# andimarafioti/faster-qwen3-tts

Measured on AMD Instinct MI355X. Metric: real-time factor (audio s / wall s), Qwen3-TTS-12Hz-0.6B voice-clone streaming chunk_size=8; p50 TTFA in ttfa_ms_p50, higher is better.
Workload: dtype bf16

## Files before the change

faster-qwen3-tts_amd/csrc/decode_kernels.cuh:

```cuda
#pragma once
#include "fq3_common.cuh"
#include <initializer_list>

namespace fq3 {

enum { PRO_PLAIN = 0, PRO_NORM = 1, PRO_COMBINE = 2 };
enum { EPI_STORE = 0, EPI_RESIDUAL = 1, EPI_SWIGLU = 2 };

constexpr int kHeadDim = 128;
constexpr int kKeysPerTile = 64;
constexpr int kMaxWorkers = 8;
constexpr int kPartStride = kHeadDim + 4;


struct GemvArgs {
    const void* W; int N; int K;
    const void* x;
    const void* norm_w; float eps;
    const void* bias;
    void* y;
    const void* res;
    void* xn_out;
    int up_off;
    const float* part; int n_part; int rep;
// ... 236 lines not shown
    a.norm_w = norm_w; a.eps = eps; a.up_off = up_off; a.n_part = n_part; a.rep = rep;
    a.bias = t.bias; a.y = t.y; a.res = t.res; a.xn_out = t.xn_out;
    a.x2 = t.x2; a.y2 = t.y2; a.res2 = t.res2; a.part_stride2 = t.part_stride2;
    gemv_body<T, NCH, PRO, EPI, NT, M, R>(a);
}
template <typename T, int NCH, int PRO, int EPI, bool NT, int M, int R>
inline void gemv_launch(const GemvArgs& a, int grid, size_t shm, hipStream_t s) {
    const GemvTail t{a.y, a.res, a.bias, a.xn_out, a.x2, a.y2, a.res2, a.part_stride2};
    const void* x = PRO == PRO_COMBINE ? static_cast<const void*>(a.part) : a.x;
    hipLaunchKernelGGL((gemv_kernel<T, NCH, PRO, EPI, NT, M, R>), dim3(grid), dim3(256), shm, s, a.W, x, a.norm_w, a.N, a.K, a.eps, a.up_off,
                       a.n_part, a.rep, t);
}

struct AttnArgs {
    const void* qkv;
    const void* q_norm_w; const void* k_norm_w; float eps;
    const float* cos_row; const float* sin_row;
    void* kcache; void* vcache; int max_seq;
    const int* table; int blk_stride;
    const int* pos_ptr; int pos_imm; int n_pad;
    const int* done_ptr;
    int n_kv; float* part; float scale;
    int rep; void* out;
};

template <typename T, int REP, bool PAGED>
__device__ __forceinline__ void attn_decode_body(const AttnArgs& a) {
    constexpr int HD = kHeadDim, KS = kKeysPerTile, NG = KS / 16;
    const int g = blockIdx.x, s = blockIdx.y, S = gridDim.y;
    __shared__ float qs[REP][HD];
    __shared__ float knew[HD], vnew[HD];
    __shared__ float wo[4][REP][HD];
    __shared__ float wm[4][REP], wl[4][REP];
    const int tid = threadIdx.x, wave = tid >> 6, lane = tid & 63;
    const int sub = lane >> 4, c = lane & 15;
    const T* qkv = reinterpret_cast<const T*>(a.qkv);
    const int q_dim = a.n_kv * REP * HD, kv_dim = a.n_kv * HD;
    T* kc = reinterpret_cast<T*>(a.kcache) + (PAGED ? (size_t)g * KS * HD : (size_t)g * a.max_seq * HD);
    T* vc = reinterpret_cast<T*>(a.vcache) + (PAGED ? (size_t)g * KS * HD : (size_t)g * a.max_seq * HD);
    const int n_tiles = (a.max_seq + KS - 1) / KS;
    auto block_of = [&](int tile) -> int {
        if constexpr (PAGED) return a.table[tile < n_tiles ? tile : n_tiles - 1];
        else return 0;
    };
    int blk = block_of(s), blk_next = block_of(s + S);

// ... 123 lines not shown
        }
    }
    __syncthreads();
    for (int e = tid; e < REP * HD; e += 256) {
        const int h = e / HD, d = e - h * HD;
        float M = fmaxf(fmaxf(wm[0][h], wm[1][h]), fmaxf(wm[2][h], wm[3][h]));
        float num = 0.f, den = 0.f;
#pragma unroll
        for (int w = 0; w < 4; ++w) {
            const float ww = __expf(wm[w][h] - M);
            num = fmaf(ww, wo[w][h][d], num);
            den = fmaf(ww, wl[w][h], den);
        }
        float* p = a.part + (((size_t)g * kMaxWorkers + s) * REP + h) * kPartStride;
        p[d] = num;
        if (d == 0) { p[HD] = M; p[HD + 1] = den; }
    }
}

struct AttnTail {
    const void* q_norm_w; const void* k_norm_w; const float* cos_row; const float* sin_row;
    const int* table; const int* pos_ptr; const int* done_ptr; float* part; void* out;
    float eps; float scale; int n_pad; int blk_stride; int rep;
};
inline AttnTail attn_tail(const AttnArgs& a) {
    return AttnTail{a.q_norm_w, a.k_norm_w, a.cos_row, a.sin_row, a.table, a.pos_ptr, a.done_ptr, a.part, a.out, a.eps, a.scale, a.n_pad, a.blk_stride, a.rep};
}
__device__ __forceinline__ AttnArgs attn_args_of(const AttnTail& t) {
    AttnArgs a;
    a.q_norm_w = t.q_norm_w; a.k_norm_w = t.k_norm_w; a.cos_row = t.cos_row; a.sin_row = t.sin_row;
    a.table = t.table; a.pos_ptr = t.pos_ptr; a.done_ptr = t.done_ptr; a.part = t.part; a.out = t.out;
    a.eps = t.eps; a.scale = t.scale; a.n_pad = t.n_pad; a.blk_stride = t.blk_stride; a.rep = t.rep;
    return a;
}

constexpr int kAttnDecodeLeadDwords = 14;
template <typename T, int REP, bool PAGED>
__global__ __launch_bounds__(256) void attn_decode_kernel(const int* table, const void* qkv, void* kcache, void* vcache, const int* pos_ptr,
                                                          int max_seq, int n_kv, int blk_stride, int pos_imm, AttnTail t) {
    AttnArgs a = attn_args_of(t);
    a.table = table; a.qkv = qkv; a.kcache = kcache; a.vcache = vcache; a.pos_ptr = pos_ptr;
    a.max_seq = max_seq; a.n_kv = n_kv; a.blk_stride = blk_stride; a.pos_imm = pos_imm;
    attn_decode_body<T, REP, PAGED>(a);
}
template <typename T, int REP, bool PAGED>
inline void attn_decode_launch(const AttnArgs& a, int workers, hipStream_t s) {
    hipLaunchKernelGGL((attn_decode_kernel<T, REP, PAGED>), dim3(a.n_kv, workers), dim3(256), 0, s, a.table, a.qkv, a.kcache, a.vcache, a.pos_ptr,
                       a.max_seq, a.n_kv, a.blk_stride, a.pos_imm, attn_tail(a));
}

template <typename T>
__device__ __forceinline__ void attn_pred_body(const AttnArgs& a, int head) {
    constexpr int HD = kHeadDim;
    const int g = head / a.rep, hh = head - g * a.rep;
    const int lane = threadIdx.x & 63, sub = lane >> 4, c = lane & 15;
    const int pos = a.pos_imm;
    const T* qkv = reinterpret_cast<const T*>(a.qkv);
    const int q_dim = a.n_kv * a.rep * HD, kv_dim = a.n_kv * HD;
    T* kc = reinterpret_cast<T*>(a.kcache) + (size_t)g * a.max_seq * HD;
    T* vc = reinterpret_cast<T*>(a.vcache) + (size_t)g * a.max_seq * HD;
    Raw8<T> qraw, knraw, vnraw, qwraw, kwraw, kr[4], vr[4];
    ldraw<false>(qraw, qkv + (size_t)head * HD + c * 8);
    ldraw<false>(knraw, qkv + q_dim + (size_t)g * HD + c * 8);
    ldraw<false>(vnraw, qkv + q_dim + kv_dim + (size_t)g * HD + c * 8);
    ldraw<false>(qwraw, reinterpret_cast<const T*>(a.q_norm_w) + c * 8);
    ldraw<false>(kwraw, reinterpret_cast<const T*>(a.k_norm_w) + c * 8);
    const f32x4 cs0 = *reinterpret_cast<const f32x4*>(a.cos_row + ((c * 8) & 63)), cs1 = *reinterpret_cast<const f32x4*>(a.cos_row + ((c * 8 + 4) & 63));
    const f32x4 sn0 = *reinterpret_cast<const f32x4*>(a.sin_row + ((c * 8) & 63)), sn1 = *reinterpret_cast<const f32x4*>(a.sin_row + ((c * 8 + 4) & 63));
#pragma unroll
    for (int i = 0; i < 4; ++i) {
        int key = i * 4 + sub;
        key = key < a.max_seq ? key : a.max_seq - 1;
        ldraw<false>(kr[i], kc + (size_t)key * HD + c * 8);
        ldraw<false>(vr[i], vc + (size_t)key * HD + c * 8);
    }
    __builtin_amdgcn_sched_barrier(0);
    const float sgn = c < 8 ? -1.f : 1.f;
    const float cs[8] = {cs0.x, cs0.y, cs0.z, cs0.w, cs1.x, cs1.y, cs1.z, cs1.w};
    const float sn[8] = {sgn * sn0.x, sgn * sn0.y, sgn * sn0.z, sgn * sn0.w, sgn * sn1.x, sgn * sn1.y, sgn * sn1.z, sgn * sn1.w};
    auto norm_rope = [&](const Raw8<T>& raw, const Raw8<T>& wraw, float (&out)[8]) {
#pragma clang fp contract(off)
        float x[8], w[8];
        unpack(raw, x); unpack(wraw, w);
        float ss = 0.f;
#pragma unroll
        for (int i = 0; i < 8; ++i) ss = fmaf(x[i], x[i], ss);
        ss = row16_sum(ss);
        const float rs = 1.0f / sqrtf(ss / (float)HD + a.eps);
#pragma unroll
        for (int i = 0; i < 8; i += 2) {
            float u = x[i] * rs, v = x[i + 1] * rs;
            DT<T>::rnd2(u, v);
            u *= w[i]; v *= w[i + 1];
            DT<T>::rnd2(u, v);
            x[i] = u; x[i + 1] = v;
        }
#pragma unroll
        for (int i = 0; i < 8; i += 2) {
// ... 319 lines not shown
```

faster-qwen3-tts_amd/csrc/fq3_api.hip:

```cpp
#define FQ3_SKINNY_EXTERN
#include "fq3_ctx.h"
#include "sampler.cuh"
#include "sampler_wave.cuh"
#include "skinny_gemm.cuh"
#include "state_kernels.cuh"

#include <cstdio>
#include <cstdlib>
#include <cstring>
#include <map>
#include <string>
#include <type_traits>
#include <vector>

using namespace fq3;

static thread_local std::string g_err;
static int fail(int code, const std::string& m) { g_err = m; return code; }
int fq3_fail_(int code, const std::string& m) { return fail(code, m); }
#define HIPCHK(x) do { hipError_t e_ = (x); if (e_ != hipSuccess) return fail(FQ3_EHIP, std::string(#x) + ": " + hipGetErrorString(e_)); } while (0)

extern "C" const char* fq3_last_error(void) { return g_err.c_str(); }
extern "C" void fq3_set_error_(const char* msg) { g_err = msg ? msg : ""; }
extern "C" int fq3_abi_version(void) { return FQ3_ABI_VERSION; }

static int dmalloc(fq3_ctx* c, void** p, size_t bytes, bool zero = true) {
    HIPCHK(hipMalloc(p, bytes));
    if (zero) HIPCHK(hipMemset(*p, 0, bytes));
    c->allocs.push_back(*p);
// ... 184 lines not shown
    if ((r = dmalloc(c, &c->act2, (size_t)Im * c->esz))) return r;
    if ((r = dmalloc(c, &c->pred_x2, (size_t)p.hidden * c->esz))) return r;
    if ((r = dmalloc(c, &c->xin, (size_t)Hm * c->esz))) return r;
    if ((r = dmalloc(c, &c->tmp_hidden, (size_t)Hm * c->esz))) return r;
    if ((r = dmalloc(c, &c->qkv, (size_t)qkvm * c->esz))) return r;
    if ((r = dmalloc(c, &c->act, (size_t)Im * c->esz))) return r;
    if ((r = dmalloc(c, &c->logits, (size_t)Vm * c->esz))) return r;
    if ((r = dmalloc(c, &c->past_hidden, (size_t)t.hidden * c->esz))) return r;
    if ((r = dmalloc(c, &c->ph_hold, (size_t)t.hidden * c->esz))) return r;
    if ((r = dmalloc(c, &c->pred_in, (size_t)2 * t.hidden * c->esz))) return r;
    if ((r = dmalloc(c, &c->pred_next, (size_t)t.hidden * c->esz))) return r;
    if ((r = dmalloc(c, &c->pred_x, (size_t)p.hidden * c->esz))) return r;
    if ((r = dmalloc(c, &c->plogits, (size_t)(G - 1) * p.vocab * c->esz))) return r;
    const int maxkv = std::max(t.n_kv_heads, p.n_kv_heads);
    c->part_stride = (size_t)maxkv * kMaxWorkers * 4 * kPartStride;
    if ((r = dmalloc(c, (void**)&c->part, 2 * c->part_stride * sizeof(float)))) return r;
    if ((r = dmalloc(c, (void**)&c->rope_now, 2 * 64 * sizeof(float)))) return r;
    if ((r = dmalloc(c, (void**)&c->seen_api, kMaxVocab))) return r;
    if ((r = dmalloc(c, (void**)&c->st, sizeof(DecodeState)))) return r;
    if ((r = dmalloc(c, (void**)&c->seen, kMaxVocab))) return r;
    if ((r = dmalloc(c, (void**)&c->codes, (size_t)(frames + 1) * G * sizeof(int)))) return r;
    if ((r = dmalloc(c, (void**)&c->ids64, (size_t)64 * sizeof(int64_t)))) return r;
    if ((r = dmalloc(c, (void**)&c->d_pemb, (size_t)64 * sizeof(void*)))) return r;
    HIPCHK(hipStreamCreateWithFlags(&c->cap_stream, hipStreamNonBlocking));
    return FQ3_OK;
}

extern "C" int fq3_set_option(fq3_ctx* c, const char* key, int value) {
    if (!c || !key) return fail(FQ3_EINVAL, "null argument");
    const std::string k(key);
    if (k == "weight_nt") c->opt_nt = value;
    else if (k == "pred_m2") c->opt_m2 = value;
    else if (k == "pred_attn") c->opt_pred_attn = value;
    else if (k == "rows_per_wave_max") c->opt_rmax = value;
    else if (k == "prefill_mode") c->prefill_mode = value;
    else if (k == "flash_prefill") c->opt_flash_prefill = value;
    else if (k == "flash_small") c->opt_flash_small = value;
    else if (k == "cont_pack") c->opt_cont_pack = value;
    else if (k == "swiglu_tile") c->opt_swiglu_tile = value;
    else if (k == "packed_weights") c->opt_packed = value;
    else if (k == "skinny_gemm") c->opt_no_skinny = !value;
    else return fail(FQ3_EINVAL, "unknown option: " + k);
    fq3_graph_reset(c);
    return FQ3_OK;
}

extern "C" int fq3_graph_reset(fq3_ctx* c) {
    if (!c) return fail(FQ3_EINVAL, "null ctx");
    if (c->exec) { (void)hipGraphExecDestroy(c->exec); c->exec = nullptr; }
    if (c->graph) { (void)hipGraphDestroy(c->graph); c->graph = nullptr; }
    return FQ3_OK;
}

namespace {
struct PackedEntry { void* p; int refs; int N, K; };
std::mutex g_packed_mu;
std::map<std::pair<const void*, int>, PackedEntry> g_packed;
// ... 35 lines not shown
        const int r = fq3_packed_acquire_(W, N, K, kind);
        if (r == FQ3_OK) c->packed_refs.emplace_back(W, kind);
        return r == FQ3_EUNSUPPORTED ? FQ3_OK : r;
    };
    auto stack = [&](const std::vector<fq3_layer_weights>& L, const fq3_stack_dims& d) -> int {
        const int qd = d.n_heads * kHeadDim, kvd = d.n_kv_heads * kHeadDim;
        for (const fq3_layer_weights& l : L) {
            if (int r = take(l.qkv, qd + 2 * kvd, d.hidden, 0)) return r;
            if (int r = take(l.o, d.hidden, qd, 0)) return r;
            if (int r = take(l.gate_up, 2 * d.inter, d.hidden, 1)) return r;
            if (int r = take(l.gate_up, 2 * d.inter, d.hidden, 0)) return r;
            if (int r = take(l.down, d.hidden, d.inter, 0)) return r;
        }
        return FQ3_OK;
    };
    if (int r = stack(c->tl, c->cfg.talker)) return r;
    if (int r = stack(c->pl, c->cfg.predictor)) return r;
    for (const fq3_layer_weights& l : c->tl) if (int r = take(l.gate_up, 2 * c->cfg.talker.inter, c->cfg.talker.hidden, 2)) return r;
    if (int r = take(c->wt.codec_head, c->cfg.talker.vocab, c->cfg.talker.hidden, 0)) return r;
    for (const void* h : c->lmh) if (int r = take(h, c->cfg.predictor.vocab, c->cfg.predictor.hidden, 0)) return r;
    return FQ3_OK;
}

extern "C" int fq3_ctx_destroy(fq3_ctx* c) {
    if (!c) return FQ3_OK;
    (void)hipDeviceSynchronize();
    fq3_graph_reset(c);
    packed_release_all(c);
    if (c->cap_stream) (void)hipStreamDestroy(c->cap_stream);
    if (fq3_kv_pool* p = c->tk.pool) {
        (void)fq3_kv_release(c, 0);
        bool last;
        { std::lock_guard<std::mutex> lk(p->mu); last = --p->users == 0; }
        if (p->is_private && last) pool_free_(p);
    }
    for (void* p : c->allocs) (void)hipFree(p);
    delete c;
    return FQ3_OK;
}

extern "C" int fq3_bind_weights(fq3_ctx* c, const fq3_weight_table* w) {
    if (!c || !w) return fail(FQ3_EINVAL, "null argument");
    const int G = c->cfg.num_code_groups;
    if (!w->talker_layers || !w->predictor_layers || !w->codec_embedding || !w->codec_head || !w->talker_final_norm ||
        !w->predictor_final_norm || !w->predictor_embeddings || !w->lm_heads || !w->talker_cos || !w->talker_sin ||
        !w->pred_cos || !w->pred_sin)
        return fail(FQ3_EINVAL, "weight table has null entries");
    if (c->cfg.has_projection && !w->proj_w) return fail(FQ3_EINVAL, "has_projection set but proj_w is null");
    if (w->talker_rope_len < c->cfg.max_seq_len || w->pred_rope_len < G + 1)
        return fail(FQ3_EINVAL, "rope tables shorter than the caches");
    c->wt = *w;
    c->tl.assign(w->talker_layers, w->talker_layers + c->cfg.talker.n_layers);
    c->pl.assign(w->predictor_layers, w->predictor_layers + c->cfg.predictor.n_layers);
    c->pemb.assign(w->predictor_embeddings, w->predictor_embeddings + (G - 1));
    c->lmh.assign(w->lm_heads, w->lm_heads + (G - 1));
    for (auto& l : c->tl) if (!l.qkv || !l.o || !l.gate_up || !l.down || !l.input_norm || !l.post_norm || !l.q_norm || !l.k_norm)
        return fail(FQ3_EINVAL, "talker layer has null weights");
    for (auto& l : c->pl) if (!l.qkv || !l.o || !l.gate_up || !l.down || !l.input_norm || !l.post_norm || !l.q_norm || !l.k_norm)
        return fail(FQ3_EINVAL, "predictor layer has null weights");
    HIPCHK(hipMemcpy(c->d_pemb, c->pemb.data(), (G - 1) * sizeof(void*), hipMemcpyHostToDevice));
    (void)hipDeviceSynchronize();
    packed_release_all(c);
    if (int r = packed_acquire_all(c)) { packed_release_all(c); return r; }
    c->bound = true;
    fq3_graph_reset(c);
    return FQ3_OK;
}

template <typename T, int NCH, int PRO, int EPI, bool NT, int M = 1>
static void launch_gemv_n(const GemvArgs& a, int rmax, hipStream_t s) {
    const int R = gemv_rows_per_wave<NCH, EPI>(a.N, rmax);
    const int grid = gemv_grid(a.N, R);
    const size_t shm = gemv_lds_bytes<PRO, M>(a.K);
    if constexpr (MaxRows<NCH, EPI>::v >= 2) {
        if (R == 2) { gemv_launch<T, NCH, PRO, EPI, NT, M, 2>(a, grid, shm, s); return; }
    }
    gemv_launch<T, NCH, PRO, EPI, NT, M, 1>(a, grid, shm, s);
}
template <typename T, int PRO, int EPI>
static int launch_gemv2_t(const GemvArgs& a, int rmax, hipStream_t s) {
    constexpr int most = gemv_most_chunks(PRO, 2);
    const int n = gemv_chunks(a.K, most);
    if (!n) return fail(FQ3_EUNSUPPORTED, PRO == PRO_NORM ? "code predictor hidden size above 2048" : "code predictor GEMV inner dimension above 3072");
    with_value<1, 2, 4, 6>(n, [&](auto nch) {
// ... 3 lines not shown
}
template <int PRO, int EPI>
static int launch_gemv2(const fq3_ctx* c, const GemvArgs& a, hipStream_t s) {
    return c->cfg.dtype == FQ3_BF16 ? launch_gemv2_t<bf16_t, PRO, EPI>(a, c->opt_rmax, s) : launch_gemv2_t<float, PRO, EPI>(a, c->opt_rmax, s);
}
template <typename T, int PRO, int EPI, bool NT>
static int launch_gemv_t(const GemvArgs& a, int rmax, hipStream_t s) {
    constexpr int most = gemv_most_chunks(PRO, 1);
    const int n = gemv_chunks(a.K, most);
    if (!n) return fail(FQ3_EUNSUPPORTED, PRO == PRO_NORM ? "hidden size above 2048" : "GEMV inner dimension above 6144");
    with_value<1, 2, 4, 6, 12>(n, [&](auto nch) {
        if constexpr (decltype(nch)::value <= most) launch_gemv_n<T, decltype(nch)::value, PRO, EPI, NT>(a, rmax, s);
    });
    return 0;
}
template <int PRO, int EPI>
static int launch_gemv(const fq3_ctx* c, const GemvArgs& a, bool nt, hipStream_t s) {
    const int rmax = c->opt_rmax;
    if (c->cfg.dtype == FQ3_BF16)
        return nt ? launch_gemv_t<bf16_t, PRO, EPI, true>(a, rmax, s) : launch_gemv_t<bf16_t, PRO, EPI, false>(a, rmax, s);
    return nt ? launch_gemv_t<float, PRO, EPI, true>(a, rmax, s) : launch_gemv_t<float, PRO, EPI, false>(a, rmax, s);
}

template <typename T, bool PAGED>
static void launch_attn_p(const AttnArgs& a, int rep, int workers, hipStream_t s) {
    with_value<1, 2, 4>(rep, [&](auto r) {
        attn_decode_launch<T, decltype(r)::value, PAGED>(a, workers, s);
    });
}
template <typename T>
static void launch_attn_t(const AttnArgs& a, int rep, int workers, hipStream_t s) {
    if (a.table) launch_attn_p<T, true>(a, rep, workers, s); else launch_attn_p<T, false>(a, rep, workers, s);
}

struct StepSrc { const void* x0; const int* pos_ptr; int pos_imm; bool kv_only_tail = false; };

static int run_stack(fq3_ctx* c, bool talker, const StepSrc& src, hipStream_t s) {
    const fq3_stack_dims& d = talker ? c->cfg.talker : c->cfg.predictor;
    const std::vector<fq3_layer_weights>& L = talker ? c->tl : c->pl;
    StackBufs& kv = talker ? c->tk : c->pk;
    const int rep = d.n_heads / d.n_kv_heads;
    const int q_dim = d.n_heads * kHeadDim, kv_dim = d.n_kv_heads * kHeadDim;
    const bool nt = c->opt_nt == 2 || (c->opt_nt == 1 && talker);
    const float *cos_row, *sin_row;
    if (src.pos_ptr) { cos_row = c->rope_now; sin_row = c->rope_now + 64; }
    else {
        const int rl = talker ? c->wt.talker_rope_len : c->wt.pred_rope_len;
        int rp = src.pos_imm + (talker ? c->rope_delta : 0);
        rp = rp < 0 ? 0 : (rp >= rl ? rl - 1 : rp);
        cos_row = (talker ? c->wt.talker_cos : c->wt.pred_cos) + (size_t)rp * 64;
        sin_row = (talker ? c->wt.talker_sin : c->wt.pred_sin) + (size_t)rp * 64;
    }
    for (int i = 0; i < d.n_layers; ++i) {
        const fq3_layer_weights& w = L[i];
        const void* xin = i == 0 ? src.x0 : c->h;
        GemvArgs g{};
        g.eps = d.rms_eps;
        g.W = w.qkv; g.N = q_dim + 2 * kv_dim; g.K = d.hidden; g.x = xin;
        g.norm_w = w.input_norm; g.y = c->qkv;
        if (int r = launch_gemv<PRO_NORM, EPI_STORE>(c, g, nt, s)) return r;
        const bool tail_skip = src.kv_only_tail && i == d.n_layers - 1;
        GemvArgs o{};
        o.W = w.o; o.N = d.hidden; o.K = q_dim; o.y = c->h; o.res = xin; o.rep = rep;
        AttnArgs a{};
        a.qkv = c->qkv; a.q_norm_w = w.q_norm; a.k_norm_w = w.k_norm; a.eps = d.rms_eps;
        a.cos_row = cos_row; a.sin_row = sin_row;
        a.kcache = kv.k[i]; a.vcache = kv.v[i]; a.max_seq = kv.max_seq;
        a.table = kv.d_table; a.blk_stride = kv.pool ? (int)kv.pool->blk_elems : 0;
        a.pos_ptr = src.pos_ptr; a.pos_imm = src.pos_imm;
        a.done_ptr = src.pos_ptr ? &c->st->done : nullptr;
        a.n_pad = talker ? c->n_pad : 0;
        a.n_kv = d.n_kv_heads; a.part = c->part;
        a.scale = 1.0f / sqrtf((float)kHeadDim);
        a.rep = rep; a.out = c->attn_out;
        const bool pred_attn = c->opt_pred_attn && !talker && !src.pos_ptr && src.pos_imm <= 16;
        if (pred_attn) {
            if (c->cfg.dtype == FQ3_BF16) attn_pred_launch<bf16_t>(a, d.n_heads, s);
            else attn_pred_launch<float>(a, d.n_heads, s);
            if (tail_skip) break;
            o.x = c->attn_out;
            if (int r = launch_gemv<PRO_PLAIN, EPI_RESIDUAL>(c, o, nt, s)) return r;
        } else {
            if (c->cfg.dtype == FQ3_BF16) launch_attn_t<bf16_t>(a, rep, kv.workers, s);
            else launch_attn_t<float>(a, rep, kv.workers, s);
            if (tail_skip) break;
            o.part = c->part; o.n_part = kv.workers;
            if (int r = launch_gemv<PRO_COMBINE, EPI_RESIDUAL>(c, o, nt, s)) return r;
        }
        GemvArgs m{};
        m.eps = d.rms_eps; m.W = w.gate_up; m.N = d.inter; m.K = d.hidden; m.x = c->h;
        m.norm_w = w.post_norm; m.y = c->act; m.up_off = d.inter;
        if (int r = launch_gemv<PRO_NORM, EPI_SWIGLU>(c, m, nt, s)) return r;
        GemvArgs dn{};
        dn.W = w.down; dn.N = d.hidden; dn.K = d.inter; dn.x = c->act; dn.y = c->h; dn.res = c->h;
        if (int r = launch_gemv<PRO_PLAIN, EPI_RESIDUAL>(c, dn, nt, s)) return r;
    }
    return 0;
// ... 370 lines not shown
        if (int r = fq3_set_generation_state(ctxs[q], 0, 0)) return r;
    if (int r = fq3_prefill_continue_batch_mfma_(ctxs, n, embeds, start, cnt, out_logits, out_hidden, s)) return r;
    LAUNCH_CHECK();
    return FQ3_OK;
}

int fq3_codec_head_launch_(fq3_ctx* c, const void* hidden, void* out_logits, hipStream_t s) {
    GemvArgs g{};
    g.W = c->wt.codec_head; g.N = c->cfg.talker.vocab; g.K = c->cfg.talker.hidden; g.x = hidden; g.y = out_logits;
    return launch_gemv<PRO_PLAIN, EPI_STORE>(c, g, true, s);
}

extern "C" int fq3_set_prefill_mode(fq3_ctx* c, int mode) { return fq3_set_option(c, "prefill_mode", mode); }

__global__ void build_seen_kernel(const int64_t* history, int n, unsigned char* seen, int V) {
    for (int i = threadIdx.x; i < V; i += blockDim.x) seen[i] = 0;
    __syncthreads();
    for (int i = threadIdx.x; i < n; i += blockDim.x) { const int id = (int)history[i]; if (id >= 0 && id < V) seen[id] = 1; }
}

template <typename T>
static void launch_sample_pred(const DecodeState* st, const T* lg, int V, int cb, const SampleCfg& cfg, const T* nz,
                               int* codes, int G, int64_t* out64, const T* next_emb, T* next_in, int H, bool wave,
                               const TeacherForcing* tf, hipStream_t s) {
    if (wave) dispatch_nc(V, [&](auto nc) {
        constexpr int NC = decltype(nc)::value;
        sample_pred_wave_launch<T, NC>(st, lg, V, cb, cfg, nz, codes, G, out64, next_emb, next_in, H, tf, s);
    });
    else hipLaunchKernelGGL((sample_pred_kernel<T>), dim3(1), dim3(256), 0, s, st, lg, V, cb, cfg, nz, codes, G, out64,
                            next_emb, next_in, H, tf);
}
template <typename T>
static void launch_sample_talker(DecodeState* st, const T* lg, int V, const unsigned char* seen, int G, bool wave,
                                 const TeacherForcing* tf, hipStream_t s) {
    if (wave) dispatch_nc(V, [&](auto nc) {
        constexpr int NC = decltype(nc)::value;
        sample_talker_wave_launch<T, NC>(st, lg, V, seen, G, tf, s);
    });
    else hipLaunchKernelGGL((sample_talker_kernel<T>), dim3(1), dim3(256), 0, s, st, lg, V, seen, G, tf);
}
template <typename T>
static void launch_sample_api(fq3_ctx* c, const T* lg, int V, const SampleCfg& cfg, const int64_t* history, int n_hist,
                              const T* noise, int64_t* out, hipStream_t s) {
    if (cfg.top_p >= 1.0f) {
        const unsigned char* seen = nullptr;
        if (n_hist > 0) {
            hipLaunchKernelGGL(build_seen_kernel, dim3(1), dim3(256), 0, s, history, n_hist, c->seen_api, V);
            seen = c->seen_api;
        }
        dispatch_nc(V, [&](auto nc) {
// ... 46 lines not shown
    if (penalty == 1.0f || n_hist <= 0 || !history) return FQ3_OK;
    hipStream_t s = (hipStream_t)stream;
    hipLaunchKernelGGL(build_seen_kernel, dim3(1), dim3(256), 0, s, history, n_hist, c->seen_api, V);
    if (c->cfg.dtype == FQ3_BF16) hipLaunchKernelGGL((rep_penalty_kernel<bf16_t>), dim3(1), dim3(256), 0, s, (bf16_t*)logits, V, c->seen_api, penalty);
    else hipLaunchKernelGGL((rep_penalty_kernel<float>), dim3(1), dim3(256), 0, s, (float*)logits, V, c->seen_api, penalty);
    LAUNCH_CHECK();
    return FQ3_OK;
}

extern "C" int fq3_set_predictor_sampling(fq3_ctx* c, const fq3_sampling* s) {
    if (!c || !s) return fail(FQ3_EINVAL, "null argument");
    if (s->do_sample && !(s->temperature > 0.f)) return fail(FQ3_EINVAL, "temperature must be > 0");
    if ((s->top_p >= 1.0f) != (c->pred_sampling.top_p >= 1.0f)) fq3_graph_reset(c);
    c->pred_sampling = *s;
    return FQ3_OK;
}

template <typename T>
static int predictor_passes_t(fq3_ctx* c, const DecodeState* st_dev, const void* pred_input, const void* noise_imm,
                              int64_t* out64, void* out_logits, hipStream_t s) {
    const fq3_stack_dims &p = c->cfg.predictor, &t = c->cfg.talker;
    const int G = c->cfg.num_code_groups, Vp = p.vocab, Ht = t.hidden;
    SampleCfg scfg = to_cfg(c->pred_sampling);
    for (int pass = 0; pass < G; ++pass) {
        const void* hsrc = c->h;
        if (pass == 0 && c->opt_m2) {
            const T* xa = (const T*)pred_input;
            const T* xb = (const T*)pred_input + Ht;
            if (c->cfg.has_projection) {
                GemvArgs g{};
                g.W = c->wt.proj_w; g.bias = c->wt.proj_b; g.N = p.hidden; g.K = Ht; g.x = xa; g.x2 = xb; g.y = c->pred_x; g.y2 = c->pred_x2;
                if (int r = launch_gemv2<PRO_PLAIN, EPI_STORE>(c, g, s)) return r;
                xa = (const T*)c->pred_x; xb = (const T*)c->pred_x2;
            }
            if (int r = run_predictor_pair(c, xa, xb, s)) return r;
            pass = 1;
            hsrc = c->h2;
        } else {
        const T* x_talker = pass < 2 ? (const T*)pred_input + (size_t)pass * Ht : (const T*)c->pred_next;
        const void* x0 = x_talker;
        if (c->cfg.has_projection) {
            GemvArgs g{};
            g.W = c->wt.proj_w; g.bias = c->wt.proj_b; g.N = p.hidden; g.K = Ht; g.x = x_talker; g.y = c->pred_x;
            if (int r = launch_gemv<PRO_PLAIN, EPI_STORE>(c, g, false, s)) return r;
            x0 = c->pred_x;
        }
        StepSrc src{x0, nullptr, pass};
        src.kv_only_tail = pass == 0;
        if (int r = run_stack(c, false, src, s)) return r;
        }
        if (pass == 0) continue;
        const int cb = pass - 1;
        T* lg = out_logits ? (T*)out_logits + (size_t)cb * Vp : (T*)c->plogits + (size_t)cb * Vp;
        GemvArgs hgm{};
        hgm.eps = p.rms_eps; hgm.W = c->lmh[cb]; hgm.N = Vp; hgm.K = p.hidden; hgm.x = hsrc;
        hgm.norm_w = c->wt.predictor_final_norm; hgm.y = lg;
        if (int r = launch_gemv<PRO_NORM, EPI_STORE>(c, hgm, false, s)) return r;
        const T* nz = noise_imm ? (const T*)noise_imm + (size_t)cb * Vp : nullptr;
        const T* next_emb = cb + 1 < G - 1 ? (const T*)c->pemb[cb] : nullptr;
        launch_sample_pred<T>(st_dev, (const T*)lg, Vp, cb, scfg, nz, st_dev ? c->codes : nullptr, G, out64, next_emb,
                              (T*)c->pred_next, Ht, c->pred_sampling.top_p >= 1.0f, st_dev ? c->tf : nullptr, s);
    }
    return 0;
}

extern "C" int fq3_predictor_loop(fq3_ctx* c, const void* pred_input, const void* noise, int64_t* out_ids,
                                  void* out_logits, void* stream) {
    NEED_BOUND(c);
    if (!pred_input || !out_ids) return fail(FQ3_EINVAL, "null argument");
    if (c->pred_sampling.do_sample && !noise) return fail(FQ3_EINVAL, "predictor sampling enabled but no noise given");
    hipStream_t s = (hipStream_t)stream;
    int r = c->cfg.dtype == FQ3_BF16 ? predictor_passes_t<bf16_t>(c, nullptr, pred_input, noise, out_ids, out_logits, s)
                                     : predictor_passes_t<float>(c, nullptr, pred_input, noise, out_ids, out_logits, s);
    if (r) return r;
    LAUNCH_CHECK();
    return FQ3_OK;
}

extern "C" int fq3_decode_begin(fq3_ctx* c, const fq3_decode_params* p, void* stream) {
    NEED_BOUND(c);
    if (!p || !p->past_hidden || !p->tts_pad_embed) return fail(FQ3_EINVAL, "null argument");
    if (p->trailing_len > 0 && !p->trailing_text) return fail(FQ3_EINVAL, "trailing_text");
    if (p->talker.do_sample && (!p->talker_noise || p->noise_frames <= 0)) return fail(FQ3_EINVAL, "talker sampling needs a noise ring");
    if (c->pred_sampling.do_sample && (!p->pred_noise || p->noise_frames <= 0)) return fail(FQ3_EINVAL, "predictor sampling needs a noise ring");
    if (p->talker.do_sample && !(p->talker.temperature > 0.f)) return fail(FQ3_EINVAL, "temperature must be > 0");
    if (p->max_new_tokens > c->cfg.max_frames) return fail(FQ3_EINVAL, "max_new_tokens exceeds the context's max_frames");
    if (p->prefill_len <= 0 || p->prefill_len > c->cfg.max_seq_len) return fail(FQ3_EINVAL, "prefill_len");
    if (p->first_token < 0 || p->first_token >= c->cfg.talker.vocab) return fail(FQ3_EINVAL, "first_token outside the codec vocabulary");
    if (p->gen_step < 0 || p->min_new_tokens < 0 || p->max_new_tokens < 0) return fail(FQ3_EINVAL, "negative counters");
    const bool wave = p->talker.top_p >= 1.0f;
    if (wave != c->talker_wave) { fq3_graph_reset(c); c->talker_wave = wave; }
    hipStream_t s = (hipStream_t)stream;
    if (int r = fq3_kv_ensure_(c, p->prefill_len + p->max_new_tokens + 1, s)) return r;
    DecodeState h{};
// ... 47 lines not shown
    tabs.t[0] = c->wt.codec_embedding;
    for (int i = 1; i < G; ++i) tabs.t[i] = c->pemb[i - 1];
    if (G != 16) return fail(FQ3_EUNSUPPORTED, "the fused loop is built for 16 code groups");
    embed_sum_launch<T, 16>(st, tabs, c->codes, (T*)c->xin, H, c->wt.talker_cos, c->wt.talker_sin, c->wt.talker_rope_len, c->rope_delta,
                            c->rope_now, s);
    StepSrc src{c->xin, &st->pos, 0};
    if (int r = run_stack(c, true, src, s)) return r;
    GemvArgs g{};
    g.eps = t.rms_eps; g.W = c->wt.codec_head; g.N = t.vocab; g.K = H; g.x = c->h;
    g.norm_w = c->wt.talker_final_norm; g.y = c->logits; g.xn_out = c->past_hidden;
    if (int r = launch_gemv<PRO_NORM, EPI_STORE>(c, g, true, s)) return r;
    launch_sample_talker<T>(st, (const T*)c->logits, t.vocab, c->seen, G, c->talker_wave, c->tf, s);
    return 0;
}
static int enqueue_frame(fq3_ctx* c, hipStream_t s) {
    return c->cfg.dtype == FQ3_BF16 ? enqueue_frame_t<bf16_t>(c, s) : enqueue_frame_t<float>(c, s);
}

extern "C" int fq3_graph_capture(fq3_ctx* c, void* stream) {
    NEED_BOUND(c);
    if (c->exec) return FQ3_OK;
    (void)stream;
    hipStream_t cs = c->cap_stream;
    HIPCHK(hipStreamBeginCapture(cs, hipStreamCaptureModeRelaxed));
    int r = enqueue_frame(c, cs);
    hipGraph_t g = nullptr;
    hipError_t e = hipStreamEndCapture(cs, &g);
    if (r) { if (g) (void)hipGraphDestroy(g); return r; }
    if (e != hipSuccess) return fail(FQ3_EHIP, std::string("hipStreamEndCapture: ") + hipGetErrorString(e));
    c->graph = g;
    HIPCHK(hipGraphInstantiate(&c->exec, c->graph, nullptr, nullptr, 0));
    return FQ3_OK;
}

extern "C" int fq3_decode_frames(fq3_ctx* c, int n_frames, void* stream) {
    NEED_BOUND(c);
    hipStream_t s = (hipStream_t)stream;
    for (int i = 0; i < n_frames; ++i) {
        if (c->exec) { HIPCHK(hipGraphLaunch(c->exec, s)); }
        else if (int r = enqueue_frame(c, s)) return r;
    }
    LAUNCH_CHECK();
    return FQ3_OK;
}

extern "C" int fq3_decode_poll(fq3_ctx* c, int* n_frames_total, int* done, void* stream) {
    if (!c) return fail(FQ3_EINVAL, "null ctx");
    hipStream_t s = (hipStream_t)stream;
    DecodeState h;
    HIPCHK(hipMemcpyAsync(&h, c->st, sizeof h, hipMemcpyDeviceToHost, s));
    HIPCHK(hipStreamSynchronize(s));
    if (n_frames_total) *n_frames_total = h.frame;
    if (done) *done = h.done == 2 ? 2 : (h.done || h.token == h.eos_id);
    return FQ3_OK;
}

extern "C" int fq3_decode_codes(fq3_ctx* c, int from, int count, int64_t* out, void* stream) {
    if (!c || !out) return fail(FQ3_EINVAL, "null argument");
    if (from < 0 || count < 0 || from + count > c->cfg.max_frames) return fail(FQ3_EINVAL, "range");
    const int G = c->cfg.num_code_groups, n = count * G;
// ... 7 lines not shown
```

faster-qwen3-tts_amd/csrc/fq3_ctx.h:

```cpp
#pragma once
#include "../../include/fq3hip.h"
#include "decode_kernels.cuh"
#include <hip/hip_runtime.h>
#include <mutex>
#include <string>
#include <utility>
#include <vector>

struct fq3_kv_pool {
    int dtype = 0, esz = 2, n_layers = 0, n_kv = 0, n_blocks = 0;
    size_t blk_elems = 0;
    std::vector<void*> k, v;
    std::vector<int> free_list;
    std::mutex mu;
    int in_use_high = 0;
    int users = 0;
    bool is_private = false;
};

struct StackBufs {
    std::vector<void*> k, v;
    int max_seq = 0, workers = 1;
    fq3_kv_pool* pool = nullptr;
    int* d_table = nullptr;
// ... 14 lines not shown
    void *pred_in = nullptr, *pred_x = nullptr, *pred_next = nullptr, *plogits = nullptr, *tmp_hidden = nullptr;
    void *attn_out = nullptr, *attn_out2 = nullptr;
    void *h2 = nullptr, *qkv2 = nullptr, *act2 = nullptr, *pred_x2 = nullptr;
    size_t part_stride = 0;
    float* part = nullptr;
    float* rope_now = nullptr;
    unsigned char* seen_api = nullptr;
    fq3::DecodeState* st = nullptr;
    fq3::TeacherForcing* tf = nullptr;
    unsigned char* seen = nullptr;
    int* codes = nullptr;
    int64_t* ids64 = nullptr;
    int n_pad = 0, rope_delta = 0;
    int opt_nt = 1;
    int opt_m2 = 1;
    int opt_pred_attn = 1;
    int opt_rmax = 2;
    int opt_flash_prefill = 1;
    int opt_flash_small = 1;
    int opt_cont_pack = 1;
    int opt_swiglu_tile = 1;
    int opt_packed = 1;
    std::vector<std::pair<const void*, int>> packed_refs;
    int opt_no_skinny = 0;
    int prefill_mode = 0;
    bool talker_wave = true;
    fq3_sampling pred_sampling{0.9f, 50, 1.0f, 1, 1.0f};
    hipGraph_t graph = nullptr;
    hipGraphExec_t exec = nullptr;
    hipStream_t cap_stream = nullptr;
    std::vector<void*> allocs;
    fq3_prompt_weights pw{};
    bool pw_bound = false;
    void *pw_x = nullptr, *pw_h = nullptr;
    int pw_cap = 0;
    void* ph_hold = nullptr;
    void *tt_tab = nullptr, *tt_x = nullptr, *tt_h = nullptr;
    int tt_alloc = 0;
    int tt_cap = 0, tt_rows = 0;
    bool tt_open = false, tt_session = false;
    bool armed = false;
    const void* begin_trailing = nullptr; int begin_trailing_len = 0;
    void *pf_x = nullptr, *pf_xn = nullptr, *pf_qkv = nullptr, *pf_att = nullptr, *pf_gu = nullptr, *pf_act = nullptr, *pf_ws = nullptr;
};


// ... 17 lines not shown
```

faster-qwen3-tts_amd/csrc/sampler_wave.cuh:

```cuda
#pragma once
#include "sampler.cuh"
#include <type_traits>

namespace fq3 {

__device__ __forceinline__ ArgMax wave_argmax(ArgMax a) {
    ArgMax r;
    r.v = wave_max(a.v);
    r.i = wave_min_i32(a.v == r.v ? a.i : 0x7fffffff);
    return r;
}

struct BlkSmem { int cnt[2][4]; float f[4]; float av[4]; int ai[4]; };

__device__ __forceinline__ float blk_max4(float v, BlkSmem& sm) {
    v = wave_max(v);
    __syncthreads();
    if ((threadIdx.x & 63) == 0) sm.f[threadIdx.x >> 6] = v;
    __syncthreads();
    return fmaxf(fmaxf(sm.f[0], sm.f[1]), fmaxf(sm.f[2], sm.f[3]));
}
__device__ __forceinline__ float blk_sum4(float v, BlkSmem& sm) {
    v = wave_sum(v);
    __syncthreads();
// ... 138 lines not shown

template <typename T, int NC>
__device__ __forceinline__ int sample_nucleus_from_regs(Raw8<T> (&xraw)[NC], int V, const SampleCfg& c, const unsigned char* seen,
                                                        const T* noise, SampleSmem& big) {
#pragma unroll
    for (int j = 0; j < NC; ++j) {
        float f[8];
        unpack(xraw[j], f);
#pragma unroll
        for (int i = 0; i < 8; ++i) {
            const int id = j * 2048 + threadIdx.x * 8 + i;
            if (id < V) big.vals[id] = f[i];
        }
    }
    __syncthreads();
    const int tok = sample_core<T>(big, V, c, seen, noise);
    __syncthreads();
    return tok;
}

template <typename T, int NC, bool NUCLEUS = false>
__device__ __forceinline__ void sample_pred_wave_body(const DecodeState* st, const T* logits, int V, int cb,
                                                      const SampleCfg& c_imm, const T* noise_imm, int* codes, int G,
                                                      int64_t* out64, const T* next_emb, T* next_in, int H, const TeacherForcing* tf = nullptr) {
    __shared__ BlkSmem sm;
    Raw8<T> xraw[NC];
    issue_logits<T, NC>(xraw, logits, V);
    SampleCfg c = c_imm;
    const T* noise = noise_imm;
    int frame = 0;
    if (st) {
        if (st->done) return;
        c.temperature = st->p_temperature; c.top_k = st->p_top_k; c.top_p = st->p_top_p; c.do_sample = st->p_do_sample;
        frame = st->frame;
        if (st->pred_noise)
            noise = gptr(reinterpret_cast<const T*>(st->pred_noise)) + ((size_t)(frame % st->noise_frames) * (G - 1) + cb) * V;
    }
    int tok;
    if constexpr (NUCLEUS) {
        __shared__ SampleSmem big;
        if (c.do_sample && c.top_p < 1.0f) tok = sample_nucleus_from_regs<T, NC>(xraw, V, c, nullptr, noise, big);
        else tok = sample_wave_core<T, NC>(xraw, V, c, nullptr, noise, sm);
    } else {
        tok = sample_wave_core<T, NC>(xraw, V, c, nullptr, noise, sm);
    }
    if (st) tok = forced_or(tf, frame * G + 1 + cb, tok);
    if (threadIdx.x == 0) {
        if (codes) codes[(size_t)frame * G + 1 + cb] = tok;
        if (out64) out64[cb] = tok;
    }
    if (next_emb) {
        const T* src = next_emb + (size_t)tok * H;
        for (int e = threadIdx.x * 8; e < H; e += 256 * 8) {
            Raw8<T> r; ldraw<false>(r, src + e);
            if (sizeof(T) == 2) *reinterpret_cast<u32x4*>(reinterpret_cast<char*>(next_in) + (size_t)e * 2) = *reinterpret_cast<u32x4*>(&r);
            else { float f[8]; unpack(r, f);
#pragma unroll
                   for (int i = 0; i < 8; ++i) DT<T>::st(next_in + e + i, f[i]); }
        }
    }
}

constexpr int kSamplePredLeadDwords = 14;
template <typename T, int NC>
__global__ __launch_bounds__(256) void sample_pred_wave_kernel(const DecodeState* st, const T* logits, const T* noise_imm, int* codes,
                                                              int64_t* out64, const T* next_emb, int V, int cb, int G, int H,
                                                              T* next_in, const TeacherForcing* tf, SampleCfg c_imm) {
    sample_pred_wave_body<T, NC>(st, logits, V, cb, c_imm, noise_imm, codes, G, out64, next_emb, next_in, H, tf);
}
template <typename T, int NC>
inline void sample_pred_wave_launch(const DecodeState* st, const T* logits, int V, int cb, const SampleCfg& c_imm, const T* noise_imm,
                                    int* codes, int G, int64_t* out64, const T* next_emb, T* next_in, int H, const TeacherForcing* tf,
                                    hipStream_t s) {
    hipLaunchKernelGGL((sample_pred_wave_kernel<T, NC>), dim3(1), dim3(256), 0, s, st, logits, noise_imm, codes, out64, next_emb, V, cb, G, H,
                       next_in, tf, c_imm);
}

template <typename T, int NC, bool NUCLEUS = false>
__device__ __forceinline__ void sample_talker_wave_body(DecodeState* st, const T* logits, int V, const unsigned char* seen, int G,
                                                        const TeacherForcing* tf = nullptr) {
    __shared__ BlkSmem sm;
    Raw8<T> xraw[NC];
    issue_logits<T, NC>(xraw, logits, V);
    if (st->done) return;
    SampleCfg c;
    c.temperature = st->t_temperature; c.top_k = st->t_top_k; c.top_p = st->t_top_p; c.do_sample = st->t_do_sample;
    c.rep_penalty = st->t_rep_penalty;
    c.sup_lo = st->sup_lo; c.sup_hi = st->sup_hi; c.keep_id = st->eos_id;
    const int frame = st->frame;
    c.sup_extra = (frame + 1 < st->min_new) ? st->eos_id : -1;
    const T* noise = st->talker_noise
        ? gptr(reinterpret_cast<const T*>(st->talker_noise)) + (size_t)(frame % st->noise_frames) * V : nullptr;
    int tok;
    if constexpr (NUCLEUS) {
        __shared__ SampleSmem big;
        if (c.do_sample && c.top_p < 1.0f) tok = sample_nucleus_from_regs<T, NC>(xraw, V, c, seen, noise, big);
        else tok = sample_wave_core<T, NC>(xraw, V, c, seen, noise, sm);
    } else {
// ... 19 lines not shown
```

Before: 38.87.

## Precompute predictor layer-0 QKV rows per codebook token and gather them at decode

Builds a device table holding the layer-0 normed QKV projection of every predictor embedding row for each codebook. During predictor passes the first layer's QKV GEMV is skipped, and the attention kernel reads the precomputed row indexed by the sampled token that the sampler now writes to a device slot. This trades a large one-time build (vocab times codebooks GEMVs) and extra memory for removing one GEMV per predictor pass. The table is weight-derived rather than activation-derived, so it is legitimate precomputation, and the prefetch order of the q/k/v loads is moved after the cache loads.

New measurement: 39.19, median of 6. No clear change (+0.8%).

```diff
diff --git a/faster-qwen3-tts_amd/csrc/decode_kernels.cuh b/faster-qwen3-tts_amd/csrc/decode_kernels.cuh
--- a/faster-qwen3-tts_amd/csrc/decode_kernels.cuh
+++ b/faster-qwen3-tts_amd/csrc/decode_kernels.cuh
@@ -282,6 +282,7 @@
     const int* done_ptr;
     int n_kv; float* part; float scale;
     int rep; void* out;
+    const int* tok_ptr; int tok_stride;
 };
 
 template <typename T, int REP, bool PAGED>
@@ -451,15 +452,18 @@
     const void* q_norm_w; const void* k_norm_w; const float* cos_row; const float* sin_row;
     const int* table; const int* pos_ptr; const int* done_ptr; float* part; void* out;
     float eps; float scale; int n_pad; int blk_stride; int rep;
+    const int* tok_ptr; int tok_stride;
 };
 inline AttnTail attn_tail(const AttnArgs& a) {
-    return AttnTail{a.q_norm_w, a.k_norm_w, a.cos_row, a.sin_row, a.table, a.pos_ptr, a.done_ptr, a.part, a.out, a.eps, a.scale, a.n_pad, a.blk_stride, a.rep};
+    return AttnTail{a.q_norm_w, a.k_norm_w, a.cos_row, a.sin_row, a.table, a.pos_ptr, a.done_ptr, a.part, a.out, a.eps, a.scale, a.n_pad, a.blk_stride, a.rep,
+                    a.tok_ptr, a.tok_stride};
 }
 __device__ __forceinline__ AttnArgs attn_args_of(const AttnTail& t) {
     AttnArgs a;
     a.q_norm_w = t.q_norm_w; a.k_norm_w = t.k_norm_w; a.cos_row = t.cos_row; a.sin_row = t.sin_row;
     a.table = t.table; a.pos_ptr = t.pos_ptr; a.done_ptr = t.done_ptr; a.part = t.part; a.out = t.out;
     a.eps = t.eps; a.scale = t.scale; a.n_pad = t.n_pad; a.blk_stride = t.blk_stride; a.rep = t.rep;
+    a.tok_ptr = t.tok_ptr; a.tok_stride = t.tok_stride;
     return a;
 }
 
@@ -485,13 +489,11 @@
     const int lane = threadIdx.x & 63, sub = lane >> 4, c = lane & 15;
     const int pos = a.pos_imm;
     const T* qkv = reinterpret_cast<const T*>(a.qkv);
+    if (a.tok_ptr) qkv += (size_t)*a.tok_ptr * a.tok_stride;
     const int q_dim = a.n_kv * a.rep * HD, kv_dim = a.n_kv * HD;
     T* kc = reinterpret_cast<T*>(a.kcache) + (size_t)g * a.max_seq * HD;
     T* vc = reinterpret_cast<T*>(a.vcache) + (size_t)g * a.max_seq * HD;
     Raw8<T> qraw, knraw, vnraw, qwraw, kwraw, kr[4], vr[4];
-    ldraw<false>(qraw, qkv + (size_t)head * HD + c * 8);
-    ldraw<false>(knraw, qkv + q_dim + (size_t)g * HD + c * 8);
-    ldraw<false>(vnraw, qkv + q_dim + kv_dim + (size_t)g * HD + c * 8);
     ldraw<false>(qwraw, reinterpret_cast<const T*>(a.q_norm_w) + c * 8);
     ldraw<false>(kwraw, reinterpret_cast<const T*>(a.k_norm_w) + c * 8);
     const f32x4 cs0 = *reinterpret_cast<const f32x4*>(a.cos_row + ((c * 8) & 63)), cs1 = *reinterpret_cast<const f32x4*>(a.cos_row + ((c * 8 + 4) & 63));
@@ -503,6 +505,9 @@
         ldraw<false>(kr[i], kc + (size_t)key * HD + c * 8);
         ldraw<false>(vr[i], vc + (size_t)key * HD + c * 8);
     }
+    ldraw<false>(qraw, qkv + (size_t)head * HD + c * 8);
+    ldraw<false>(knraw, qkv + q_dim + (size_t)g * HD + c * 8);
+    ldraw<false>(vnraw, qkv + q_dim + kv_dim + (size_t)g * HD + c * 8);
     __builtin_amdgcn_sched_barrier(0);
     const float sgn = c < 8 ? -1.f : 1.f;
     const float cs[8] = {cs0.x, cs0.y, cs0.z, cs0.w, cs1.x, cs1.y, cs1.z, cs1.w};
diff --git a/faster-qwen3-tts_amd/csrc/fq3_api.hip b/faster-qwen3-tts_amd/csrc/fq3_api.hip
--- a/faster-qwen3-tts_amd/csrc/fq3_api.hip
+++ b/faster-qwen3-tts_amd/csrc/fq3_api.hip
@@ -5,6 +5,7 @@
 #include "skinny_gemm.cuh"
 #include "state_kernels.cuh"
 
+#include <algorithm>
 #include <cstdio>
 #include <cstdlib>
 #include <cstring>
@@ -235,9 +236,12 @@
     if ((r = dmalloc(c, (void**)&c->codes, (size_t)(frames + 1) * G * sizeof(int)))) return r;
     if ((r = dmalloc(c, (void**)&c->ids64, (size_t)64 * sizeof(int64_t)))) return r;
     if ((r = dmalloc(c, (void**)&c->d_pemb, (size_t)64 * sizeof(void*)))) return r;
+    if ((r = dmalloc(c, (void**)&c->entry_tok, sizeof(int)))) return r;
     HIPCHK(hipStreamCreateWithFlags(&c->cap_stream, hipStreamNonBlocking));
     return FQ3_OK;
 }
+
+static void entry_release(fq3_ctx* c);
 
 extern "C" int fq3_set_option(fq3_ctx* c, const char* key, int value) {
     if (!c || !key) return fail(FQ3_EINVAL, "null argument");
@@ -245,7 +249,8 @@
     if (k == "weight_nt") c->opt_nt = value;
     else if (k == "pred_m2") c->opt_m2 = value;
     else if (k == "pred_attn") c->opt_pred_attn = value;
-    else if (k == "rows_per_wave_max") c->opt_rmax = value;
+    else if (k == "rows_per_wave_max") { c->opt_rmax = value; entry_release(c); }
+    else if (k == "pred_entry") c->opt_pred_entry = value;
     else if (k == "prefill_mode") c->prefill_mode = value;
     else if (k == "flash_prefill") c->opt_flash_prefill = value;
     else if (k == "flash_small") c->opt_flash_small = value;
@@ -327,10 +332,60 @@
     return FQ3_OK;
 }
 
+namespace {
+struct EntryTable {
+    void* p; int refs;
+    int rmax, n_cb, Vp, hidden, row_elems; float eps;
+    const void* norm; std::vector<const void*> pemb;
+};
+std::mutex g_entry_mu;
+std::map<const void*, EntryTable> g_entry;
+}
+static int entry_build_(fq3_ctx* c, void* table);
+static void entry_release(fq3_ctx* c) {
+    if (c->entry) {
+        std::lock_guard<std::mutex> lk(g_entry_mu);
+        auto it = g_entry.find(c->entry_key);
+        if (it != g_entry.end() && --it->second.refs <= 0) { (void)hipFree(it->second.p); g_entry.erase(it); }
+    }
+    c->entry = nullptr; c->entry_key = nullptr; c->entry_tried = false;
+}
+static bool entry_eligible(const fq3_ctx* c) {
+    const fq3_stack_dims& p = c->cfg.predictor;
+    return c->opt_pred_entry && c->cfg.dtype == FQ3_BF16 && !c->cfg.has_projection && p.hidden == c->cfg.talker.hidden &&
+           c->cfg.num_code_groups >= 3;
+}
+static void entry_ensure(fq3_ctx* c, hipStream_t s) {
+    if (c->entry || c->entry_tried || !c->bound || !entry_eligible(c)) return;
+    hipStreamCaptureStatus cap = hipStreamCaptureStatusNone;
+    if (s && (hipStreamIsCapturing(s, &cap) != hipSuccess || cap != hipStreamCaptureStatusNone)) { (void)hipGetLastError(); return; }
+    const fq3_stack_dims& p = c->cfg.predictor;
+    const int n_cb = c->cfg.num_code_groups - 2, row_elems = (p.n_heads + 2 * p.n_kv_heads) * kHeadDim;
+    const void* key = c->pl[0].qkv;
+    std::lock_guard<std::mutex> lk(g_entry_mu);
+    c->entry_tried = true;
+    auto it = g_entry.find(key);
+    if (it != g_entry.end()) {
+        EntryTable& e = it->second;
+        if (e.rmax != c->opt_rmax || e.n_cb != n_cb || e.Vp != p.vocab || e.hidden != p.hidden || e.row_elems != row_elems ||
+            e.eps != p.rms_eps || e.norm != c->pl[0].input_norm || !std::equal(e.pemb.begin(), e.pemb.end(), c->pemb.begin())) return;
+        ++e.refs;
+        c->entry = e.p; c->entry_key = key;
+        return;
+    }
+    void* tab = nullptr;
+    if (hipMalloc(&tab, (size_t)n_cb * p.vocab * row_elems * 2) != hipSuccess) { (void)hipGetLastError(); return; }
+    if (entry_build_(c, tab)) { (void)hipFree(tab); (void)hipGetLastError(); return; }
+    g_entry[key] = EntryTable{tab, 1, c->opt_rmax, n_cb, p.vocab, p.hidden, row_elems, p.rms_eps, c->pl[0].input_norm,
+                              std::vector<const void*>(c->pemb.begin(), c->pemb.begin() + n_cb)};
+    c->entry = tab; c->entry_key = key;
+}
+
 extern "C" int fq3_ctx_destroy(fq3_ctx* c) {
     if (!c) return FQ3_OK;
     (void)hipDeviceSynchronize();
     fq3_graph_reset(c);
+    entry_release(c);
     packed_release_all(c);
     if (c->cap_stream) (void)hipStreamDestroy(c->cap_stream);
     if (fq3_kv_pool* p = c->tk.pool) {
@@ -365,6 +420,7 @@
         return fail(FQ3_EINVAL, "predictor layer has null weights");
     HIPCHK(hipMemcpy(c->d_pemb, c->pemb.data(), (G - 1) * sizeof(void*), hipMemcpyHostToDevice));
     (void)hipDeviceSynchronize();
+    entry_release(c);
     packed_release_all(c);
     if (int r = packed_acquire_all(c)) { packed_release_all(c); return r; }
     c->bound = true;
@@ -414,6 +470,27 @@
     return nt ? launch_gemv_t<float, PRO, EPI, true>(a, rmax, s) : launch_gemv_t<float, PRO, EPI, false>(a, rmax, s);
 }
 
+static int entry_build_(fq3_ctx* c, void* table) {
+    const fq3_stack_dims& p = c->cfg.predictor;
+    const int n_cb = c->cfg.num_code_groups - 2, row_elems = (p.n_heads + 2 * p.n_kv_heads) * kHeadDim;
+    hipStream_t bs = nullptr;
+    HIPCHK(hipStreamCreateWithFlags(&bs, hipStreamNonBlocking));
+    int r = 0;
+    for (int cb = 0; cb < n_cb && !r; ++cb)
+        for (int tok = 0; tok < p.vocab && !r; ++tok) {
+            GemvArgs g{};
+            g.eps = p.rms_eps; g.W = c->pl[0].qkv; g.N = row_elems; g.K = p.hidden; g.norm_w = c->pl[0].input_norm;
+            g.x = (const char*)c->pemb[cb] + (size_t)tok * p.hidden * 2;
+            g.y = (char*)table + ((size_t)cb * p.vocab + tok) * row_elems * 2;
+            r = launch_gemv<PRO_NORM, EPI_STORE>(c, g, false, bs);
+        }
+    const hipError_t e1 = hipGetLastError(), e2 = hipStreamSynchronize(bs);
+    (void)hipStreamDestroy(bs);
+    if (r) return r;
+    if (e1 != hipSuccess || e2 != hipSuccess) return fail(FQ3_EHIP, "building the predictor entry table failed");
+    return 0;
+}
+
 template <typename T, bool PAGED>
 static void launch_attn_p(const AttnArgs& a, int rep, int workers, hipStream_t s) {
     with_value<1, 2, 4>(rep, [&](auto r) {
@@ -425,7 +502,7 @@
     if (a.table) launch_attn_p<T, true>(a, rep, workers, s); else launch_attn_p<T, false>(a, rep, workers, s);
 }
 
-struct StepSrc { const void* x0; const int* pos_ptr; int pos_imm; bool kv_only_tail = false; };
+struct StepSrc { const void* x0; const int* pos_ptr; int pos_imm; bool kv_only_tail = false; const void* entry_rows = nullptr; };
 
 static int run_stack(fq3_ctx* c, bool talker, const StepSrc& src, hipStream_t s) {
     const fq3_stack_dims& d = talker ? c->cfg.talker : c->cfg.predictor;
@@ -450,7 +527,8 @@
         g.eps = d.rms_eps;
         g.W = w.qkv; g.N = q_dim + 2 * kv_dim; g.K = d.hidden; g.x = xin;
         g.norm_w = w.input_norm; g.y = c->qkv;
-        if (int r = launch_gemv<PRO_NORM, EPI_STORE>(c, g, nt, s)) return r;
+        const bool from_table = src.entry_rows && i == 0;
+        if (!from_table) if (int r = launch_gemv<PRO_NORM, EPI_STORE>(c, g, nt, s)) return r;
         const bool tail_skip = src.kv_only_tail && i == d.n_layers - 1;
         GemvArgs o{};
         o.W = w.o; o.N = d.hidden; o.K = q_dim; o.y = c->h; o.res = xin; o.rep = rep;
@@ -465,6 +543,7 @@
         a.n_kv = d.n_kv_heads; a.part = c->part;
         a.scale = 1.0f / sqrtf((float)kHeadDim);
         a.rep = rep; a.out = c->attn_out;
+        if (from_table) { a.qkv = src.entry_rows; a.tok_ptr = c->entry_tok; a.tok_stride = g.N; }
         const bool pred_attn = c->opt_pred_attn && !talker && !src.pos_ptr && src.pos_imm <= 16;
         if (pred_attn) {
             if (c->cfg.dtype == FQ3_BF16) attn_pred_launch<bf16_t>(a, d.n_heads, s);
@@ -881,10 +960,10 @@
 template <typename T>
 static void launch_sample_pred(const DecodeState* st, const T* lg, int V, int cb, const SampleCfg& cfg, const T* nz,
                                int* codes, int G, int64_t* out64, const T* next_emb, T* next_in, int H, bool wave,
-                               const TeacherForcing* tf, hipStream_t s) {
+                               const TeacherForcing* tf, hipStream_t s, int* tok_out = nullptr) {
     if (wave) dispatch_nc(V, [&](auto nc) {
         constexpr int NC = decltype(nc)::value;
-        sample_pred_wave_launch<T, NC>(st, lg, V, cb, cfg, nz, codes, G, out64, next_emb, next_in, H, tf, s);
+        sample_pred_wave_launch<T, NC>(st, lg, V, cb, cfg, nz, codes, G, out64, next_emb, next_in, H, tf, s, tok_out);
     });
     else hipLaunchKernelGGL((sample_pred_kernel<T>), dim3(1), dim3(256), 0, s, st, lg, V, cb, cfg, nz, codes, G, out64,
                             next_emb, next_in, H, tf);
@@ -977,6 +1056,8 @@
     const fq3_stack_dims &p = c->cfg.predictor, &t = c->cfg.talker;
     const int G = c->cfg.num_code_groups, Vp = p.vocab, Ht = t.hidden;
     SampleCfg scfg = to_cfg(c->pred_sampling);
+    const bool use_entry = c->entry && entry_eligible(c) && c->opt_pred_attn && c->pred_sampling.top_p >= 1.0f;
+    const void* entry_rows = nullptr;
     for (int pass = 0; pass < G; ++pass) {
         const void* hsrc = c->h;
         if (pass == 0 && c->opt_m2) {
@@ -1002,6 +1083,7 @@
         }
         StepSrc src{x0, nullptr, pass};
         src.kv_only_tail = pass == 0;
+        src.entry_rows = entry_rows;
         if (int r = run_stack(c, false, src, s)) return r;
         }
         if (pass == 0) continue;
@@ -1013,8 +1095,10 @@
         if (int r = launch_gemv<PRO_NORM, EPI_STORE>(c, hgm, false, s)) return r;
         const T* nz = noise_imm ? (const T*)noise_imm + (size_t)cb * Vp : nullptr;
         const T* next_emb = cb + 1 < G - 1 ? (const T*)c->pemb[cb] : nullptr;
+        entry_rows = use_entry && next_emb && cb + 2 <= 16
+            ? (const char*)c->entry + (size_t)cb * Vp * (p.n_heads + 2 * p.n_kv_heads) * kHeadDim * sizeof(T) : nullptr;
         launch_sample_pred<T>(st_dev, (const T*)lg, Vp, cb, scfg, nz, st_dev ? c->codes : nullptr, G, out64, next_emb,
-                              (T*)c->pred_next, Ht, c->pred_sampling.top_p >= 1.0f, st_dev ? c->tf : nullptr, s);
+                              (T*)c->pred_next, Ht, c->pred_sampling.top_p >= 1.0f, st_dev ? c->tf : nullptr, s, entry_rows ? c->entry_tok : nullptr);
     }
     return 0;
 }
@@ -1025,6 +1109,7 @@
     if (!pred_input || !out_ids) return fail(FQ3_EINVAL, "null argument");
     if (c->pred_sampling.do_sample && !noise) return fail(FQ3_EINVAL, "predictor sampling enabled but no noise given");
     hipStream_t s = (hipStream_t)stream;
+    entry_ensure(c, s);
     int r = c->cfg.dtype == FQ3_BF16 ? predictor_passes_t<bf16_t>(c, nullptr, pred_input, noise, out_ids, out_logits, s)
                                      : predictor_passes_t<float>(c, nullptr, pred_input, noise, out_ids, out_logits, s);
     if (r) return r;
@@ -1118,6 +1203,7 @@
     if (c->exec) return FQ3_OK;
     (void)stream;
     hipStream_t cs = c->cap_stream;
+    entry_ensure(c, cs);
     HIPCHK(hipStreamBeginCapture(cs, hipStreamCaptureModeRelaxed));
     int r = enqueue_frame(c, cs);
     hipGraph_t g = nullptr;
@@ -1132,6 +1218,7 @@
 extern "C" int fq3_decode_frames(fq3_ctx* c, int n_frames, void* stream) {
     NEED_BOUND(c);
     hipStream_t s = (hipStream_t)stream;
+    if (!c->exec) entry_ensure(c, s);
     for (int i = 0; i < n_frames; ++i) {
         if (c->exec) { HIPCHK(hipGraphLaunch(c->exec, s)); }
         else if (int r = enqueue_frame(c, s)) return r;
diff --git a/faster-qwen3-tts_amd/csrc/fq3_ctx.h b/faster-qwen3-tts_amd/csrc/fq3_ctx.h
--- a/faster-qwen3-tts_amd/csrc/fq3_ctx.h
+++ b/faster-qwen3-tts_amd/csrc/fq3_ctx.h
@@ -60,6 +60,11 @@
     int opt_swiglu_tile = 1;
     int opt_packed = 1;
     std::vector<std::pair<const void*, int>> packed_refs;
+    int opt_pred_entry = 1;
+    const void* entry = nullptr;
+    const void* entry_key = nullptr;
+    int* entry_tok = nullptr;
+    bool entry_tried = false;
     int opt_no_skinny = 0;
     int prefill_mode = 0;
     bool talker_wave = true;
diff --git a/faster-qwen3-tts_amd/csrc/sampler_wave.cuh b/faster-qwen3-tts_amd/csrc/sampler_wave.cuh
--- a/faster-qwen3-tts_amd/csrc/sampler_wave.cuh
+++ b/faster-qwen3-tts_amd/csrc/sampler_wave.cuh
@@ -184,7 +184,8 @@
 template <typename T, int NC, bool NUCLEUS = false>
 __device__ __forceinline__ void sample_pred_wave_body(const DecodeState* st, const T* logits, int V, int cb,
                                                       const SampleCfg& c_imm, const T* noise_imm, int* codes, int G,
-                                                      int64_t* out64, const T* next_emb, T* next_in, int H, const TeacherForcing* tf = nullptr) {
+                                                      int64_t* out64, const T* next_emb, T* next_in, int H, const TeacherForcing* tf = nullptr,
+                                                      int* tok_out = nullptr) {
     __shared__ BlkSmem sm;
     Raw8<T> xraw[NC];
     issue_logits<T, NC>(xraw, logits, V);
@@ -210,6 +211,7 @@
     if (threadIdx.x == 0) {
         if (codes) codes[(size_t)frame * G + 1 + cb] = tok;
         if (out64) out64[cb] = tok;
+        if (tok_out) *tok_out = tok;
     }
     if (next_emb) {
         const T* src = next_emb + (size_t)tok * H;
@@ -223,19 +225,20 @@
     }
 }
 
+struct SamplePredTail { SampleCfg c_imm; int* tok_out; };
 constexpr int kSamplePredLeadDwords = 14;
 template <typename T, int NC>
 __global__ __launch_bounds__(256) void sample_pred_wave_kernel(const DecodeState* st, const T* logits, const T* noise_imm, int* codes,
                                                               int64_t* out64, const T* next_emb, int V, int cb, int G, int H,
-                                                              T* next_in, const TeacherForcing* tf, SampleCfg c_imm) {
-    sample_pred_wave_body<T, NC>(st, logits, V, cb, c_imm, noise_imm, codes, G, out64, next_emb, next_in, H, tf);
+                                                              T* next_in, const TeacherForcing* tf, SamplePredTail t) {
+    sample_pred_wave_body<T, NC>(st, logits, V, cb, t.c_imm, noise_imm, codes, G, out64, next_emb, next_in, H, tf, t.tok_out);
 }
 template <typename T, int NC>
 inline void sample_pred_wave_launch(const DecodeState* st, const T* logits, int V, int cb, const SampleCfg& c_imm, const T* noise_imm,
                                     int* codes, int G, int64_t* out64, const T* next_emb, T* next_in, int H, const TeacherForcing* tf,
-                                    hipStream_t s) {
+                                    hipStream_t s, int* tok_out = nullptr) {
     hipLaunchKernelGGL((sample_pred_wave_kernel<T, NC>), dim3(1), dim3(256), 0, s, st, logits, noise_imm, codes, out64, next_emb, V, cb, G, H,
-                       next_in, tf, c_imm);
+                       next_in, tf, SamplePredTail{c_imm, tok_out});
 }
 
 template <typename T, int NC, bool NUCLEUS = false>
```
